# blyssprivacy/sdk

Measured on NVIDIA H100. Metric: PIR server queries/sec (Spiral process_query), higher is better.
Workload: dtype u64

## Files before the change

sdk_b200/csrc/api.cu:

```cuda
#include "../../include/b200pir.h"
#include "kernels.h"
#include "ntt_tables.hpp"
#include "update_body.hpp"
#include "dpir_wire.hpp"
#include "gadget.hpp"
#include <cstdio>
#include <cerrno>
#include <fcntl.h>
#include <unistd.h>
#include <algorithm>
#include <cmath>
#include <memory>
#include <cstring>
#include <condition_variable>
#include <chrono>
#include <deque>
#include <mutex>
#include <set>
#include <string>
#include <utility>
#include <vector>

using namespace b200pir;

// ... 41 lines not shown
  void ensure(size_t count) { if (count > n) alloc(count); }
  void release() { if (p) cudaFree(p); p = nullptr; n = 0; }
  ~DevBuf() { release(); }
  DevBuf(const DevBuf&) = delete;
  DevBuf& operator=(const DevBuf&) = delete;
};

enum Stage { ST_EXPAND = 0, ST_MUL, ST_FROMNTT, ST_FOLD, ST_PACK, ST_ENCODE, ST_QIMG , ST_COUNT };

}

struct b200pir_ctx {
  int device = 0;
  cudaStream_t stream = nullptr;
  bool own_stream = true;
  std::recursive_mutex mu;
  b200pir_params hp;
  int dim0, num_per, slices, trials, g, stop_round, num_packing;
  int bits_gsw, bits_conv, bits_left, bits_right;
  int live_gsw, live_conv, live_left, live_right;
  bool has_right;
  uint64_t q2, q1, setup_bytes, query_bytes, response_bytes;
  int q1_bits;
  DevParams dp;
  DevBuf<Twiddle> d_tw;
  DevBuf<Twiddle> d_tw4k;
  DevBuf<uint32_t> d_neg1;
  int mul_variant = 0, max_group = 16, profile = 0;
  int sparse_fold = 0;
  int db_format = -1;
  DevBuf<uint2> w_qf;
  DevBuf<uint8_t> w_qt;
  int sm_count = 0;
  size_t ws_queries = 0, ws_rows = 0;
  DevBuf<uint64_t> w_query;
  DevBuf<uint32_t> w_v;
  DevBuf<uint32_t> w_zflags;
  DevBuf<uint32_t> w_xr;
  DevBuf<uint4> w_qdev;
  DevBuf<uint32_t> w_vfold, w_vfold_neg;
  DevBuf<uint32_t> w_mult;
  DevBuf<uint32_t> w_cts;
  const uint32_t* folded = nullptr;
  size_t folded_stride = 0;
  DevBuf<uint64_t> w_packed;
  DevBuf<uint8_t> w_resp;
  static constexpr size_t kWriteStageBytes = (size_t)64 << 20;
  static constexpr size_t kWriteStageItems = 65536;
  DevBuf<uint8_t> w_wbytes;
  DevBuf<ItemWrite> w_witems;
  std::mutex export_mu;
  uint8_t* h_export[2] = {nullptr, nullptr};
  size_t h_export_bytes = 0;
  cudaEvent_t export_done[2] = {nullptr, nullptr};
  void ensure_export_staging(size_t bytes) {
    w_wbytes.ensure(std::max(kWriteStageBytes, bytes));
    if (!export_done[0])
      for (auto& e : export_done) B200_CUDA(cudaEventCreateWithFlags(&e, cudaEventDisableTiming | cudaEventBlockingSync));
    if (bytes <= h_export_bytes) return;
    release_export_pinned();
    const size_t n = std::max(kWriteStageBytes, bytes);
    for (auto& h : h_export) B200_CUDA(cudaHostAlloc(reinterpret_cast<void**>(&h), n, cudaHostAllocDefault));
    h_export_bytes = n;
  }
  void release_export_pinned() {
    for (auto& h : h_export) { if (h) cudaFreeHost(h); h = nullptr; }
// ... 240 lines not shown
}

void run_expand_query(b200pir_ctx* c, b200pir_pp* pp, const uint64_t* query_raw, uint32_t* v, uint4* q_dev,
                      uint32_t* v_fold, int nq, uint8_t* images = nullptr) {
  const auto& hp = c->hp;
  cudaStream_t s = c->stream;
  launch_to_ntt_strided(c->dp, v, c->v_words(), query_raw, (size_t)2 * POLY, 2, nq, s);
  run_coefficient_expansion(c, pp, v, c->v_words(), nq, false);
  const int factor = hp.nu_2 > 0 ? 2 : 1;
  if (images) {
    const Tc5Geom T = make_tc5_geom(c->dim0, 32);
    for (int q0 = 0; q0 < nq; q0 += 16)
      launch_reorient_to_tc5(T, v + (size_t)q0 * c->v_words(), c->v_words(), factor, std::min(16, nq - q0),
                             images + (size_t)(q0 / 16) * tc5_query_bytes(T), s);
  } else {
    launch_reorient(c->geom(c->num_per), q_dev, (size_t)c->dim0 * POLY, v, c->v_words(), nq, factor, s);
  }
  if (hp.nu_2 > 0)
    launch_regev_to_gsw(c->dp, v_fold, c->fold_words(), v, c->v_words(), nq, (int)hp.nu_2, 2, 1, c->pp_table(pp, (size_t)nq).conv,
                        (int)hp.t_gsw, (int)hp.t_conv, c->bits_conv, c->live_conv, s);
}

void run_fold(b200pir_ctx* c, uint64_t* cts, size_t batch, size_t batch_stride, size_t num, int k0,
              const uint32_t* vfold, const uint32_t* vfold_neg, int slices_per_query) {
  const size_t mat = (size_t)2 * 2 * c->hp.t_gsw * 2 * POLY;
  int k = k0;
  for (size_t half = num / 2; half >= 1; half /= 2, k--) {
    launch_fold_round(c->dp, cts, batch, batch_stride, (int)half, vfold + (size_t)k * mat, vfold_neg + (size_t)k * mat,
                      c->fold_words(), slices_per_query, (int)c->hp.t_gsw, c->bits_gsw, c->stream);
  }
}

const uint32_t* run_fold_res(b200pir_ctx* c, uint32_t* a, uint32_t* b, size_t batch, size_t batch_stride, size_t num,
                             int k0, const uint32_t* vfold, int slices_per_query) {
  const size_t mat = (size_t)2 * 2 * c->hp.t_gsw * 2 * POLY;
  int k = k0;
  uint32_t* src = a;
  uint32_t* dst = b;
  uint32_t* zero_flags = nullptr;
  if (c->sparse_fold) {
    c->w_zflags.ensure(batch * num);
    zero_flags = c->w_zflags.p;
  }
  for (size_t half = num / 2; half >= 1; half /= 2, k--) {
    launch_fold_res(c->dp, src, dst, batch, batch_stride, (int)half, vfold + (size_t)k * mat, c->fold_words(),
                    slices_per_query, (int)c->hp.t_gsw, c->bits_gsw, c->live_gsw, zero_flags, c->stream);
    std::swap(src, dst);
  }
  return src;
}

void run_prepare(b200pir_ctx* c, b200pir_pp* pp, size_t count, bool images = false) {
  b200pir_ctx::Scope sc(c, ST_EXPAND);
  if (images) c->w_qt.ensure((count + 15) / 16 * tc5_query_bytes(make_tc5_geom(c->dim0, 32)));
  if (c->hp.expand_queries)
    run_expand_query(c, pp, c->w_query.p, c->w_v.p, c->w_qdev.p, c->w_vfold.p, (int)count, images ? c->w_qt.p : nullptr);
}

void run_first_dim(b200pir_ctx* c, b200pir_db* db, size_t count, const uint4* qdev, uint32_t* out, int slice_begin,
                   int slice_count, const uint8_t* images = nullptr, size_t per_group = 16) {
  const DbLayout& L = db->layout;
  const size_t q_stride = (size_t)c->dim0 * POLY;
  const size_t out_stride = (size_t)c->slices * db->rows * 4 * POLY;
  if (L.format == 0) {
    b200pir_ctx::Scope sc(c, ST_MUL);
    size_t qi = 0;
    while (qi < count) {
      int nq = 1;
      if (count - qi >= 4 && c->max_group >= 4) nq = 4;
      else if (count - qi >= 2 && c->max_group >= 2) nq = 2;
      launch_multiply(c->dp, L.G, reinterpret_cast<const uint4*>(L.base), qdev + qi * q_stride, out + qi * out_stride,
                      slice_begin, slice_count, nq, q_stride, out_stride, c->mul_variant, c->stream);
      c->mul_launches++;
      qi += nq;
    }
  } else if (L.format == 2) {
    if (!images) c->w_qt.ensure(tc5_query_bytes(L.T));
    const size_t step = images ? per_group : 16;
    for (size_t qi = 0, g = 0; qi < count; qi += step, g++) {
      const int nq = (int)std::min<size_t>(step, count - qi);
      const uint8_t* qt = images ? images + g * tc5_query_bytes(L.T) : c->w_qt.p;
      if (!images) {
        b200pir_ctx::Scope sq(c, ST_QIMG);
        launch_query_to_tc5(L.T, qdev + qi * q_stride, q_stride, nq, c->w_qt.p, c->stream);
      }
      b200pir_ctx::Scope sc(c, ST_MUL);
      launch_multiply_tc5(c->dp, L.T, L.base, db->tile_mask.p, qt, out + qi * out_stride, out_stride, nq, slice_begin,
                          slice_count, c->sm_count, c->stream);
      c->mul_launches++;
    }
  } else {
    c->w_qf.ensure(imma_query_cells(L.F));
    const size_t per_pass = (c->max_group >= 16 && imma_supports_16(L.F)) ? 16 : (c->max_group >= 8 ? 8 : 4);
    for (size_t qi = 0; qi < count; qi += per_pass) {
      const int nq = (int)std::min<size_t>(per_pass, count - qi);
      {
        b200pir_ctx::Scope sq(c, ST_QIMG);
        launch_query_to_frag(L.F, qdev + qi * q_stride, q_stride, nq, c->w_qf.p, c->stream);
      }
      {
        b200pir_ctx::Scope sc(c, ST_MUL);
        launch_multiply_imma(c->dp, L.F, reinterpret_cast<const uint4*>(L.base), c->w_qf.p, out + qi * out_stride, out_stride,
                             nq, slice_begin, slice_count, c->stream);
        c->mul_launches++;
      }
    }
  }
}

void run_first_dim_and_fold(b200pir_ctx* c, b200pir_db* db, size_t count, const uint4* qdev = nullptr,
                            const uint32_t* vfold = nullptr, const uint8_t* images = nullptr, size_t per_group = 16) {
  if (!qdev) qdev = c->w_qdev.p;
  if (!vfold) vfold = c->w_vfold.p;
  const int rows = db->rows;
  const size_t out_stride = (size_t)c->slices * rows * 4 * POLY;
  const bool zmajor = db->zmajor_product();
  run_first_dim(c, db, count, qdev, zmajor ? c->w_cts.p : c->w_mult.p, 0, c->slices, images, per_group);
  {
    b200pir_ctx::Scope sc(c, ST_FROMNTT);
    if (zmajor) launch_intt_from_zmajor(c->dp, db->layout.F, c->w_cts.p, out_stride, c->w_mult.p, (int)count, c->slices, c->stream);
    else launch_ntt32(c->dp, c->w_mult.p, count * c->slices * rows * 2, true, c->stream);
  }
  {
    b200pir_ctx::Scope sc(c, ST_FOLD);
    c->folded = c->w_mult.p;
    c->folded_stride = (size_t)rows * 4 * POLY;
    if (rows > 1)
      c->folded = run_fold_res(c, c->w_mult.p, c->w_cts.p, count * c->slices, (size_t)rows * 4 * POLY, rows,
                               (int)c->hp.nu_2 - 1, vfold, c->slices);
  }
}

void run_pack_encode(b200pir_ctx* c, b200pir_pp* pp, const uint32_t* folded, size_t ct_stride, size_t count,
                     uint8_t* out_dev) {
  const auto& hp = c->hp;
  const size_t packed_words = (size_t)hp.instances * (hp.n + 1) * hp.n * POLY;
  {
    b200pir_ctx::Scope sc(c, ST_PACK);
    launch_pack(c->dp, c->w_packed.p, packed_words, folded, ct_stride, (size_t)c->slices * ct_stride, (int)count, c->pp_table(pp, count).pack,
                (int)hp.n, (int)hp.instances, (int)hp.t_conv, c->bits_conv, c->live_conv, (int)hp.version, c->stream);
  }
  {
    b200pir_ctx::Scope sc(c, ST_ENCODE);
    launch_encode(c->dp, out_dev, c->response_bytes, c->w_packed.p, packed_words, (int)count, (int)hp.n, (int)hp.instances,
                  c->q2, (int)hp.q2_bits, c->q1, c->q1_bits, c->stream);
  }
}

bool same_params(const b200pir_ctx* a, const b200pir_ctx* b) {
  return a == b || (a->device == b->device && std::memcmp(&a->hp, &b->hp, sizeof(b200pir_params)) == 0);
}
void check_db(b200pir_ctx* c, b200pir_db* db) {
  if (!db || !same_params(db->ctx, c)) throw Error(B200PIR_E_BADARG, "db handle was created for different parameters / device");
}
void check_pp(b200pir_ctx* c, b200pir_pp* pp) {
  if (!pp || !same_params(pp->ctx, c)) throw Error(B200PIR_E_BADARG, "pp handle was created for different parameters / device");
}

}

extern "C" {

// ... 89 lines not shown
  dp.q[0] = (uint32_t)q0; dp.q[1] = (uint32_t)q1m;
  dp.cr1[0] = (uint64_t)(((u128)1 << 64) / q0);
  dp.cr1[1] = (uint64_t)(((u128)1 << 64) / q1m);
  dp.modulus = q0 * q1m;
  dp.cr1_mod = (uint64_t)(((u128)1 << 64) / dp.modulus);
  dp.q1_inv_mod_q0 = (uint32_t)invmod(q1m % q0, q0);
  dp.fwd[0] = c->d_tw.p; dp.inv[0] = c->d_tw.p + POLY; dp.fwd[1] = c->d_tw.p + 2 * POLY; dp.inv[1] = c->d_tw.p + 3 * POLY;
  dp.inv_lz[0] = c->d_tw.p + 4 * POLY; dp.inv_lz[1] = c->d_tw.p + 5 * POLY;
  dp.mu58[0] = (uint32_t)(((uint64_t)1 << 58) / q0); dp.mu58[1] = (uint32_t)(((uint64_t)1 << 58) / q1m);
  {
    std::vector<uint32_t> h((size_t)NTT_LOG_N * 2 * POLY, 0);
    for (int i = 0; i < NTT_LOG_N; i++) {
      int idx = POLY - (1 << i);
      h[((size_t)i * 2 + 0) * POLY + idx] = (uint32_t)(q0 - 1);
      h[((size_t)i * 2 + 1) * POLY + idx] = (uint32_t)(q1m - 1);
    }
    c->d_neg1.alloc(h.size());
    B200_CUDA(cudaMemcpy(c->d_neg1.p, h.data(), h.size() * 4, cudaMemcpyHostToDevice));
    launch_ntt32(dp, c->d_neg1.p, NTT_LOG_N, false, c->stream);
    B200_CUDA(cudaStreamSynchronize(c->stream));
  }
  B200_CUDA(cudaGetLastError());
  *out = c.release();
  API_END
}

void b200pir_ctx_destroy(b200pir_ctx* c) {
  if (!c) return;
  cudaSetDevice(c->device);
  cudaDeviceSynchronize();
  for (auto e : c->event_pool) cudaEventDestroy(e);
  c->release_export_pinned();
  for (auto e : c->export_done) if (e) cudaEventDestroy(e);
  if (c->own_stream && c->stream) cudaStreamDestroy(c->stream);
  delete c;
}
int b200pir_ctx_set_stream(b200pir_ctx* c, void* cuda_stream) {
  API_BEGIN
  if (!c) throw Error(B200PIR_E_BADARG, "null ctx");
  Guard gd(c);
  B200_CUDA(cudaStreamSynchronize(c->stream));
  if (c->own_stream && c->stream) cudaStreamDestroy(c->stream);
  c->stream = (cudaStream_t)cuda_stream;
  c->own_stream = false;
  API_END
}
int b200pir_ctx_synchronize(b200pir_ctx* c) {
  API_BEGIN
  if (!c) throw Error(B200PIR_E_BADARG, "null ctx");
  Guard gd(c);
  B200_CUDA(cudaStreamSynchronize(c->stream));
  B200_CUDA(cudaGetLastError());
  API_END
}
int b200pir_ctx_reserve(b200pir_ctx* c, size_t queries, size_t rows_local) {
  API_BEGIN
  if (!c) throw Error(B200PIR_E_BADARG, "null ctx");
  if (queries == 0 || queries > 4096 || rows_local == 0 || rows_local > ((size_t)1 << c->hp.nu_2))
    throw Error(B200PIR_E_BADARG, "reserve: 1..4096 queries, 1..num_per rows");
  Guard gd(c);
  B200_CUDA(cudaStreamSynchronize(c->stream));
  c->ensure_workspace(queries, rows_local);
  B200_CUDA(cudaGetLastError());
  API_END
}
int b200pir_ctx_set_option(b200pir_ctx* c, const char* key, int64_t value) {
  API_BEGIN
  if (!c || !key) throw Error(B200PIR_E_BADARG, "null argument");
  Guard gd(c);
  std::string k(key);
  if (k == "mul_variant") c->mul_variant = (int)value;
  else if (k == "batch") { if (value != 1 && value != 2 && value != 4 && value != 8 && value != 16) throw Error(B200PIR_E_BADARG, "batch must be 1, 2, 4, 8 or 16"); c->max_group = (int)value; }
  else if (k == "fold_variant" || k == "intt_variant" || k == "imma_variant" || k == "expand_variant" ||
           k == "expand_pair_min_ctas") {}
  else if (k == "sparse_fold") c->sparse_fold = value != 0;
  else if (k == "coalesce") c->coalesce = value != 0;
  else if (k == "coalesce_window_us") { if (value < 0 || value > 100000) throw Error(B200PIR_E_BADARG, "coalesce_window_us must be 0..100000"); c->coalesce_window_us = (int)value; }
  else if (k == "db_format") { if (value < -1 || value > 2) throw Error(B200PIR_E_BADARG, "db_format must be -1 (automatic), 0, 1 or 2"); c->db_format = (int)value; }
  else if (k == "profile") {
    if (value < 0 || value > 2) throw Error(B200PIR_E_BADARG, "profile must be 0, 1 or 2");
    c->profile = (int)value;
    c->spans.clear(); c->event_next = 0; c->mul_launches = 0;
  }
  else throw Error(B200PIR_E_BADARG, "unknown option " + k);
  API_END
}
int b200pir_ctx_sizes(b200pir_ctx* c, uint64_t* setup_bytes, uint64_t* query_bytes, uint64_t* response_bytes) {
  API_BEGIN
  if (!c) throw Error(B200PIR_E_BADARG, "null ctx");
  if (setup_bytes) *setup_bytes = c->setup_bytes;
  if (query_bytes) *query_bytes = c->query_bytes;
  if (response_bytes) *response_bytes = c->response_bytes;
  API_END
}

int b200pir_db_create(b200pir_ctx* c, uint64_t shard_index, uint64_t shard_count, b200pir_db** out) {
  API_BEGIN
  if (!c || !out) throw Error(B200PIR_E_BADARG, "null argument");
  Guard gd(c);
  if (shard_count == 0) { shard_count = 1; shard_index = 0; }
  if (shard_index >= shard_count || (shard_count & (shard_count - 1)) || (uint64_t)c->num_per % shard_count)
    throw Error(B200PIR_E_BADARG, "shard_count must be a power of two dividing num_per");
  std::unique_ptr<b200pir_db> db(new b200pir_db());
  db->ctx = c;
  db->shard = Shard{(int)shard_index, (int)shard_count};
  db->rows = c->num_per / (int)shard_count;
  DbLayout& L = db->layout;
  L.G = c->geom(db->rows);
// ... 472 lines not shown
  if (count == 0) return 0;
  DevBuf<uint64_t> d(count * 2 * POLY);
  B200_CUDA(cudaMemcpyAsync(d.p, polys, d.n * 8, cudaMemcpyHostToDevice, c->stream));
  launch_ntt_u64(c->dp, d.p, count, inverse, c->stream);
  B200_CUDA(cudaMemcpyAsync(polys, d.p, d.n * 8, cudaMemcpyDeviceToHost, c->stream));
  B200_CUDA(cudaStreamSynchronize(c->stream));
  B200_CUDA(cudaGetLastError());
  API_END
}
int b200pir_ntt_forward(b200pir_ctx* c, uint64_t* polys, size_t count) { return ntt_host(c, polys, count, false); }
int b200pir_ntt_inverse(b200pir_ctx* c, uint64_t* polys, size_t count) { return ntt_host(c, polys, count, true); }

int b200pir_ntt32_dev(b200pir_ctx* c, uint32_t* polys_dev, size_t count, int inverse) {
  API_BEGIN
  if (!c || !polys_dev) throw Error(B200PIR_E_BADARG, "null argument");
  Guard gd(c);
  launch_ntt32(c->dp, polys_dev, count, inverse != 0, c->stream);
  B200_CUDA(cudaGetLastError());
  API_END
}

namespace {
const Twiddle* tables_4k(b200pir_ctx* c) {
  if (!c->d_tw4k.p) {
    const int N = 4096, LG = 12;
    std::vector<Twiddle> all;
    for (int n = 0; n < 2; n++) {
      std::vector<Twiddle> f, i;
      build_tables(c->dp.q[n], f, i, N, LG);
      all.insert(all.end(), f.begin(), f.end());
      all.insert(all.end(), i.begin(), i.end());
    }
    c->d_tw4k.alloc(all.size());
    B200_CUDA(cudaMemcpy(c->d_tw4k.p, all.data(), all.size() * sizeof(Twiddle), cudaMemcpyHostToDevice));
  }
  return c->d_tw4k.p;
}
}
int b200pir_ntt4096_dev(b200pir_ctx* c, uint32_t* polys_dev, size_t count, int inverse) {
  API_BEGIN
  if (!c || !polys_dev) throw Error(B200PIR_E_BADARG, "null argument");
  Guard gd(c);
  launch_ntt32_4k(c->dp.q[0], c->dp.q[1], tables_4k(c), polys_dev, count, inverse != 0, c->stream);
  B200_CUDA(cudaGetLastError());
  API_END
}
int b200pir_ntt4096(b200pir_ctx* c, uint64_t* polys, size_t count, int inverse) {
  API_BEGIN
  if (!c || (!polys && count)) throw Error(B200PIR_E_BADARG, "null argument");
  Guard gd(c);
  if (count == 0) return 0;
  const size_t words = count * 2 * 4096;
  DevBuf<uint64_t> wide(words);
  DevBuf<uint32_t> nar(words);
  B200_CUDA(cudaMemcpyAsync(wide.p, polys, words * 8, cudaMemcpyHostToDevice, c->stream));
  launch_narrow(nar.p, wide.p, words, c->stream);
  launch_ntt32_4k(c->dp.q[0], c->dp.q[1], tables_4k(c), nar.p, count, inverse != 0, c->stream);
  launch_widen(wide.p, nar.p, words, c->stream);
  B200_CUDA(cudaMemcpyAsync(polys, wide.p, words * 8, cudaMemcpyDeviceToHost, c->stream));
  B200_CUDA(cudaStreamSynchronize(c->stream));
  B200_CUDA(cudaGetLastError());
  API_END
}

int b200pir_to_ntt(b200pir_ctx* c, uint64_t* out_ntt, const uint64_t* raw, size_t count) {
  API_BEGIN
  if (!c || !out_ntt || !raw) throw Error(B200PIR_E_BADARG, "null argument");
// ... 1234 lines not shown
```

sdk_b200/csrc/kernels.h:

```cpp
#pragma once
#include "common.cuh"
#include "item_place.cuh"

namespace b200pir {

extern thread_local unsigned long long g_kernel_launches;

void opt_in_smem_impl(const void* kernel, int bytes);
template <typename K>
inline void opt_in_smem(K* kernel, int bytes) { opt_in_smem_impl(reinterpret_cast<const void*>(kernel), bytes); }

void launch_ntt_u64(const DevParams& P, uint64_t* polys, size_t count, bool inverse, cudaStream_t s);
void launch_ntt32(const DevParams& P, uint32_t* polys, size_t count, bool inverse, cudaStream_t s);
void launch_ntt32_4k(uint32_t q0, uint32_t q1, const Twiddle* tw, uint32_t* polys, size_t count, bool inverse, cudaStream_t s);
void launch_to_ntt(const DevParams& P, uint32_t* out, const uint64_t* raw, size_t count, cudaStream_t s);
void launch_to_ntt_strided(const DevParams& P, uint32_t* out, size_t out_stride, const uint64_t* raw, size_t raw_stride,
                           size_t count, int batches, cudaStream_t s);
void launch_chacha_first_rows(uint64_t* raw, const uint8_t seed[32], uint64_t word0, uint32_t n_mats, uint32_t row_words,
                              uint64_t mat_words, uint64_t modulus, cudaStream_t s);
void launch_direct_query_to_dev(uint4* q_dev, const uint32_t* sig_ntt, const uint64_t* wire_words, int dim0, cudaStream_t s);
void launch_from_ntt(const DevParams& P, uint64_t* out_raw, const uint32_t* in, size_t count, cudaStream_t s);
void launch_raw_to_res(const DevParams& P, uint32_t* out, const uint64_t* raw, size_t polys, cudaStream_t s);
void launch_res_to_raw(const DevParams& P, uint64_t* out, const uint32_t* res, size_t polys, cudaStream_t s);
void upload_poly_constants(const Twiddle* lo );
void upload_mul_constants(const Twiddle* lo );
void launch_widen(uint64_t* out, const uint32_t* in, size_t words, cudaStream_t s);
void launch_narrow(uint32_t* out, const uint64_t* in, size_t words, cudaStream_t s);

void launch_multiply(const DevParams& P, const MulGeom& G, const uint4* db_dev, const uint4* q_dev, uint32_t* out,
                     int slice_begin, int slice_count, int nq, size_t q_stride, size_t out_stride, int variant,
                     cudaStream_t s);
void launch_query_to_dev(const MulGeom& G, uint4* q_dev, const uint64_t* v_firstdim, cudaStream_t s);
struct Shard { int index, count; };
void launch_db_retile_chunk(const MulGeom& G, Shard sh, uint4* db_dev_slice, const uint64_t* ref_chunk, int z0, int zc,
                            cudaStream_t s);
void launch_db_synth(const DevParams& P, const MulGeom& G, Shard sh, uint4* db_dev, uint64_t seed, uint64_t pt_modulus,
                     int slice_begin, int slice_count, cudaStream_t s);

size_t imma_query_cells(const ImmaGeom& F);
bool imma_supports_16(const ImmaGeom& F);
inline int imma_query_tiles(int nq) { return nq > 8 ? 4 : (nq > 4 ? 2 : 1); }
void upload_imma_constants(const Twiddle* lo);
void launch_db_to_frag(const ImmaGeom& F, const uint4* db0_slice, uint4* dbf, int slice, cudaStream_t s);
void launch_query_to_frag(const ImmaGeom& F, const uint4* q_dev, size_t q_stride, int nq, uint2* qf, cudaStream_t s);
void launch_multiply_imma(const DevParams& P, const ImmaGeom& F, const uint4* dbf, const uint2* qf, uint32_t* out_zm,
                          size_t out_stride, int nq, int slice_begin, int slice_count, cudaStream_t s);
void launch_intt_from_zmajor(const DevParams& P, const ImmaGeom& F, const uint32_t* in_zm, size_t in_stride, uint32_t* out,
                             int nq, int slices, cudaStream_t s);
void launch_zmajor_to_ntt32(const ImmaGeom& F, const uint32_t* in_zm, uint32_t* out, int slice, cudaStream_t s);

size_t tc5_query_bytes(const Tc5Geom& T);
bool tc5_supported(const Tc5Geom& T);
void launch_db_to_tc5(const Tc5Geom& T, const uint4* db0_slice, uint8_t* dbt, int slice, cudaStream_t s);
void launch_query_to_tc5(const Tc5Geom& T, const uint4* q_dev, size_t q_stride, int nq, uint8_t* qt, cudaStream_t s);
void launch_reorient_to_tc5(const Tc5Geom& T, const uint32_t* v, size_t v_stride, int idx_factor, int nq, uint8_t* qt, cudaStream_t s);
void launch_multiply_tc5(const DevParams& P, const Tc5Geom& T, const uint8_t* dbt, const uint32_t* tile_mask, const uint8_t* qt,
                         uint32_t* out_zm, size_t out_stride, int nq, int slice_begin, int slice_count, int sm_count, cudaStream_t s);

void launch_db_upsert(const DbLayout& L, int slice, int il, int j, const uint64_t* poly, cudaStream_t s);
struct ItemWrite { uint32_t off, len, il, j; };
void launch_write_items(const DevParams& P, const DbLayout& L, const uint8_t* bytes, const ItemWrite* items, int count, int chunks,
                        int bpc, uint64_t pt_modulus, cudaStream_t s);
void launch_db_export(const DbLayout& L, int slice, int z0, int zc, uint64_t* out, cudaStream_t s);

void launch_fold_round(const DevParams& P, uint64_t* cts, size_t batch, size_t batch_stride , int half,
                       const uint32_t* c_pos, const uint32_t* c_neg, size_t c_batch_stride ,
                       int slices_per_query, int t_gsw, int bits, cudaStream_t s);
void launch_fold_res(const DevParams& P, const uint32_t* in, uint32_t* out, size_t batch, size_t batch_stride ,
                     int half, const uint32_t* c_pos, size_t c_batch_stride, int slices_per_query, int t_gsw, int bits, int live,
                     uint32_t* zero_flags , cudaStream_t s);
void launch_folding_neg(const DevParams& P, uint32_t* out, const uint32_t* v_folding, int count, int t_gsw, int bits,
                        cudaStream_t s);

struct PpTable { const uint32_t* const* pack; const uint32_t* const* left; const uint32_t* const* right; const uint32_t* const* conv; };
struct ExpandRound {
  int r, num_in, stop_round, max_bits_to_gen_right, t_auto;
  const uint32_t* const* tab_left;
  const uint32_t* const* tab_right;
  size_t off_left, off_right;
  int t_left, t_right, bits_left, bits_right;
  int live_left, live_right;
  int fill_skipped;
};
void launch_expand_round_res(const DevParams& P, uint32_t* v, size_t v_stride, uint32_t* xr, size_t xr_stride, int nq,
                             const ExpandRound& R, const uint32_t* neg1_r, cudaStream_t s);
void launch_reorient(const MulGeom& G, uint4* q_dev, size_t q_stride, const uint32_t* v, size_t v_stride, int nq,
                     int idx_factor, cudaStream_t s);
void launch_regev_to_gsw(const DevParams& P, uint32_t* v_gsw, size_t gsw_stride, const uint32_t* v, size_t v_stride,
                         int nq, int count, int idx_factor, int idx_offset, const uint32_t* const* tab_conv, int t_gsw,
                         int t_conv, int bits_conv, int live_conv, cudaStream_t s);
// ... 40 lines not shown
```

sdk_b200/csrc/tc5_kernels.cu:

```cuda
#include "kernels.h"
#include "item_place.cuh"
#include "tc5_ptx.cuh"

namespace b200pir {

namespace {

constexpr int TC5_SMEM_BUDGET = 227 * 1024 - 1024;
constexpr int TC5_THREADS = 2 * 128 + 32;

using namespace tc5;

__global__ void __launch_bounds__(256)
k_db_to_tc5(Tc5Geom T, const uint4* __restrict__ db0_slice, uint8_t* __restrict__ dbt, int slice) {
  const int z = blockIdx.x, mt = blockIdx.y, ks = blockIdx.z;
  const Tc5DbThread t = tc5_db_thread(threadIdx.x, mt, ks);
  const int half = T.dim0 >> 1;
  uint32_t res[2][4];
#pragma unroll
  for (int p = 0; p < 2; p++) {
    const int jp = t.jp0 + p;
    uint4 w = make_uint4(0, 0, 0, 0);
    if (t.ii < T.rows && jp < half) w = db0_slice[((size_t)t.ii * half + jp) * POLY + z];
    res[0][2 * p] = w.x; res[1][2 * p] = w.y; res[0][2 * p + 1] = w.z; res[1][2 * p + 1] = w.w;
// ... 48 lines not shown
  __syncthreads();
#pragma unroll
  for (int zz = 0; zz < 8; zz++)
#pragma unroll
    for (int n = 0; n < 2; n++) {
      uint4* dst = reinterpret_cast<uint4*>(qt + tc5_q_tile(T, n, z0 + zz, ks) * TC5_TILE);
      dst[threadIdx.x] = reinterpret_cast<const uint4*>(rimg + ((size_t)zz * 2 + n) * TC5_TILE)[threadIdx.x];
    }
}

constexpr int TC5_MAX_STAGES = 24;
struct Tc5Smem {
  uint64_t full[TC5_MAX_STAGES], empty[TC5_MAX_STAGES];
  uint64_t bfull[2], bempty[2];
};
__host__ __device__ inline int tc5_ring_stages(int ks, int ksps, int bbufs) {
  const int n = (TC5_SMEM_BUDGET - bbufs * ks * TC5_TILE) / (ksps * TC5_TILE);
  return n > TC5_MAX_STAGES ? TC5_MAX_STAGES : n;
}

template <int KSPS, int BBUFS>
__global__ void __launch_bounds__(TC5_THREADS, 1)
k_multiply_tc5(DevParams P, Tc5Geom T, const uint8_t* __restrict__ dbt, const uint8_t* __restrict__ qt,
               uint32_t* __restrict__ out_zm, size_t out_stride, int nq, int slice_begin, int slice_count,
               const uint32_t* __restrict__ tile_mask ) {
  constexpr int TC5_STAGE_BYTES = KSPS * TC5_TILE;
  const int TC5_STAGES = tc5_ring_stages(T.ks, KSPS, BBUFS);
  extern __shared__ __align__(1024) uint8_t tc5_smem[];
  uint8_t* smem_b = tc5_smem;
  uint8_t* smem_a = smem_b + (size_t)BBUFS * T.ks * TC5_TILE;
  Tc5Smem* S = reinterpret_cast<Tc5Smem*>(smem_a + (size_t)TC5_STAGES * TC5_STAGE_BYTES);
  const int warp = threadIdx.x >> 5, lane = threadIdx.x & 31;
  const int stages_per_tile = (T.ks + KSPS - 1) / KSPS;
  const int tiles_per_item = slice_count * T.mt;
  const int n_items = 2 * POLY;
  const uint32_t b_bytes = (uint32_t)T.ks * TC5_TILE;

  if (threadIdx.x == 0) {
    for (int s = 0; s < TC5_STAGES; s++) { mbar_init(&S->full[s], 1); mbar_init(&S->empty[s], 2); }
    for (int b = 0; b < 2; b++) { mbar_init(&S->bfull[b], 1); mbar_init(&S->bempty[b], 2); }
    asm volatile("fence.mbarrier_init.release.cluster;" ::: "memory");
  }
  __syncthreads();

  if (warp == 8) {
    int stage = 0; uint32_t sphase = 0;
    int it = 0;
    for (int item = blockIdx.x; item < n_items; item += gridDim.x, it++) {
      const int n = item & 1, z = item >> 1, bb = it % BBUFS;
      mbar_wait(&S->bempty[bb], ((it / BBUFS) & 1) ^ 1);
      if (elect_one()) {
        mbar_expect_tx(&S->bfull[bb], b_bytes);
        bulk_g2s(smem_b + (size_t)bb * b_bytes, qt + tc5_q_tile(T, n, z, 0) * TC5_TILE, b_bytes, &S->bfull[bb]);
      }
      __syncwarp();
      for (int sl = 0; sl < slice_count; sl++)
        for (int mt = 0; mt < T.mt; mt++) {
          const uint8_t* src = dbt + tc5_db_tile(T, slice_begin + sl, n, z, mt, 0) * TC5_TILE;
          const uint32_t mask = __ldg(tile_mask + (size_t)(slice_begin + sl) * T.mt + mt);
          for (int st = 0; st < stages_per_tile; st++) {
            const int ks_here = min(KSPS, T.ks - st * KSPS);
            const uint32_t full_m = ks_here == 32 ? 0xffffffffu : ((1u << ks_here) - 1u);
            const uint32_t km = (mask >> (st * KSPS)) & full_m;
            if (km == 0) continue;
            mbar_wait(&S->empty[stage], sphase ^ 1);
            if (elect_one()) {
              uint8_t* dst = smem_a + (size_t)stage * TC5_STAGE_BYTES;
              const uint8_t* from = src + (size_t)st * TC5_STAGE_BYTES;
              mbar_expect_tx(&S->full[stage], (uint32_t)__popc(km) * TC5_TILE);
              if (km == full_m) bulk_g2s(dst, from, (uint32_t)ks_here * TC5_TILE, &S->full[stage]);
              else
                for (int kk = 0; kk < ks_here; kk++)
                  if ((km >> kk) & 1u) bulk_g2s(dst + (size_t)kk * TC5_TILE, from + (size_t)kk * TC5_TILE, TC5_TILE, &S->full[stage]);
            }
            __syncwarp();
            if (++stage == TC5_STAGES) { stage = 0; sphase ^= 1; }
          }
        }
    }
  } else if (warp < 8) {
    const int wg = warp >> 2, w = warp & 3;
    const bool leader = (threadIdx.x & 127) == 0;
    int stage = 0; uint32_t sphase = 0;
    int it = 0;
    for (int item = blockIdx.x; item < n_items; item += gridDim.x, it++) {
      const int n = item & 1, z = item >> 1, bb = it % BBUFS;
      const uint32_t q = n ? P.q[1] : P.q[0];
      const Tc5Weights W = tc5_lane_weights(lane, q);
      mbar_wait(&S->bfull[bb], (it / BBUFS) & 1);
      const uint32_t b_addr = smem_u32(smem_b + (size_t)bb * b_bytes);
      for (int t = 0, slice = slice_begin, mt = 0; t < tiles_per_item; t++, mt++) {
        if (mt == T.mt) { mt = 0; slice++; }
        const uint32_t mask = __ldg(tile_mask + (size_t)slice * T.mt + mt);
        uint32_t acc[64];
#pragma unroll
        for (int c = 0; c < 64; c++) acc[c] = 0;
        int prev = -1;
        for (int st = 0; st < stages_per_tile; st++) {
          const int ks_here = min(KSPS, T.ks - st * KSPS);
          const uint32_t km = (mask >> (st * KSPS)) & (ks_here == 32 ? 0xffffffffu : ((1u << ks_here) - 1u));
          if (km == 0) continue;
          mbar_wait(&S->full[stage], sphase);
          const uint32_t a_addr = smem_u32(smem_a + (size_t)stage * TC5_STAGE_BYTES) + wg * (TC5_TILE / 2);
          wgmma_fence();
#pragma unroll
          for (int kk = 0; kk < KSPS; kk++)
            if ((km >> kk) & 1u)
              wgmma_m64n128k32_u8(acc, tc5_smem_desc(a_addr + kk * TC5_TILE), tc5_smem_desc(b_addr + (st * KSPS + kk) * TC5_TILE));
          wgmma_commit();
          wgmma_wait<1>();
          if (prev >= 0 && leader) mbar_arrive(&S->empty[prev]);
          prev = stage;
          if (++stage == TC5_STAGES) { stage = 0; sphase ^= 1; }
        }
        wgmma_wait<0>();
        wgmma_fence_operands(acc);
        if (prev >= 0 && leader) mbar_arrive(&S->empty[prev]);
        uint64_t p32[32], s16[16], k16[16], s8[8], k8[8], s4[4], k4[4];
#pragma unroll
        for (int i = 0; i < 16; i++)
#pragma unroll
          for (int h = 0; h < 2; h++) p32[2 * i + h] = tc5_lane_partial(acc[4 * i + 2 * h], acc[4 * i + 2 * h + 1], W.w, W.wp);
        tc5_rs_split<32>((lane >> tc5_rs_lane_bit(0)) & 1, p32, s16, k16);
#pragma unroll
// ... 11 lines not shown
            out_zm[(size_t)qi * out_stride + ((((size_t)slice * 2 + n) * POLY + z) * T.rows + ii) * 2 + tc5_frag_ctrow(lane)] =
                tc5_barrett57(k4[f], W.mu, q);
        }
      }
      if (leader) mbar_arrive(&S->bempty[bb]);
    }
  }
}

}

size_t tc5_query_bytes(const Tc5Geom& T) { return (size_t)2 * POLY * T.ks * TC5_TILE; }
static size_t tc5_smem_bytes(const Tc5Geom& T, int ksps, int bbufs) {
  return (size_t)bbufs * T.ks * TC5_TILE + (size_t)tc5_ring_stages(T.ks, ksps, bbufs) * ksps * TC5_TILE + sizeof(Tc5Smem) + 16;
}
bool tc5_supported(const Tc5Geom& T) { return T.dim0 % 2 == 0 && tc5_ring_stages(T.ks, 4, 1) >= 2; }

void launch_db_to_tc5(const Tc5Geom& T, const uint4* db0_slice, uint8_t* dbt, int slice, cudaStream_t s) {
  ++g_kernel_launches;
  k_db_to_tc5<<<dim3(POLY, T.mt, T.ks), 256, 0, s>>>(T, db0_slice, dbt, slice);
}
void launch_query_to_tc5(const Tc5Geom& T, const uint4* q_dev, size_t q_stride, int nq, uint8_t* qt, cudaStream_t s) {
  if (nq < 1 || nq > 16) throw Error(-2, "wgmma multiply: 1..16 queries per pass");
  ++g_kernel_launches;
  k_query_to_tc5<<<dim3(POLY / 2, T.ks), 256, 0, s>>>(T, q_dev, q_stride, nq, qt);
}
void launch_reorient_to_tc5(const Tc5Geom& T, const uint32_t* v, size_t v_stride, int idx_factor, int nq, uint8_t* qt, cudaStream_t s) {
  if (nq < 1 || nq > 16) throw Error(-2, "wgmma multiply: 1..16 queries per pass");
  ++g_kernel_launches;
  opt_in_smem(k_reorient_to_tc5, 16 * TC5_TILE);
  k_reorient_to_tc5<<<dim3(POLY / 8, T.ks), 256, 16 * TC5_TILE, s>>>(T, v, v_stride, idx_factor, nq, qt);
}
void launch_multiply_tc5(const DevParams& P, const Tc5Geom& T, const uint8_t* dbt, const uint32_t* tile_mask, const uint8_t* qt,
                         uint32_t* out_zm, size_t out_stride, int nq, int slice_begin, int slice_count, int sm_count, cudaStream_t s) {
  if (nq < 1 || nq > 16) throw Error(-2, "wgmma multiply: 1..16 queries per pass");
  if (!tc5_supported(T)) throw Error(-2, "wgmma multiply: dim0 too large for one CTA's shared memory");
  ++g_kernel_launches;
  const int grid = sm_count > 0 ? (sm_count < 2 * POLY ? sm_count : 2 * POLY) : 132;
  int ksps = 8, bbufs = 2;
  if (tc5_ring_stages(T.ks, ksps, bbufs) < 2) ksps = 4;
  if (tc5_ring_stages(T.ks, ksps, bbufs) < 2) bbufs = 1;
  const size_t smem = tc5_smem_bytes(T, ksps, bbufs);
#define TC5_LAUNCH(K, B)                                                                                                       \
  do {                                                                                                                         \
    opt_in_smem(k_multiply_tc5<K, B>, 227 * 1024);                                                                             \
    k_multiply_tc5<K, B><<<grid, TC5_THREADS, smem, s>>>(P, T, dbt, qt, out_zm, out_stride, nq, slice_begin, slice_count, tile_mask); \
  } while (0)
  if (ksps == 4) { if (bbufs == 2) TC5_LAUNCH(4, 2); else TC5_LAUNCH(4, 1); }
  else { if (bbufs == 2) TC5_LAUNCH(8, 2); else TC5_LAUNCH(8, 1); }
#undef TC5_LAUNCH
}

}
```

Measured before the change: 1580.

## Split tail work items across CTAs and overlap iNTT/fold halves on side stream

The tc5 multiply kernel now splits the leftover work items (those that do not fill a whole wave of the grid) into tile segments, so the last wave is spread across all CTAs rather than leaving most of them idle. The first-dim pipeline splits the query batch in half and runs the second half's iNTT and fold on a side stream synchronized by events, which aims to let the two halves run concurrently. New knobs for CTA count, slice groups and B-buffer count are also added. The side stream adds event overhead and partial-tile segments reload the query B tile for each segment.

```diff
diff --git a/sdk_b200/csrc/api.cu b/sdk_b200/csrc/api.cu
--- a/sdk_b200/csrc/api.cu
+++ b/sdk_b200/csrc/api.cu
@@ -97,6 +97,17 @@
   DevBuf<uint2> w_qf;
   DevBuf<uint8_t> w_qt;
   int sm_count = 0;
+  int first_dim_ctas = 0;
+  int first_dim_slice_groups = 0;
+  int first_dim_bbufs = 0;
+  cudaStream_t side_stream = nullptr;
+  cudaEvent_t side_begin = nullptr, side_end = nullptr;
+  void ensure_side_stream() {
+    if (side_stream) return;
+    B200_CUDA(cudaStreamCreateWithFlags(&side_stream, cudaStreamNonBlocking));
+    B200_CUDA(cudaEventCreateWithFlags(&side_begin, cudaEventDisableTiming));
+    B200_CUDA(cudaEventCreateWithFlags(&side_end, cudaEventDisableTiming));
+  }
   size_t ws_queries = 0, ws_rows = 0;
   DevBuf<uint64_t> w_query;
   DevBuf<uint32_t> w_v;
@@ -403,19 +414,21 @@
 }
 
 const uint32_t* run_fold_res(b200pir_ctx* c, uint32_t* a, uint32_t* b, size_t batch, size_t batch_stride, size_t num,
-                             int k0, const uint32_t* vfold, int slices_per_query) {
+                             int k0, const uint32_t* vfold, int slices_per_query, cudaStream_t st = nullptr,
+                             size_t flags_at = 0) {
+  if (!st) st = c->stream;
   const size_t mat = (size_t)2 * 2 * c->hp.t_gsw * 2 * POLY;
   int k = k0;
   uint32_t* src = a;
   uint32_t* dst = b;
   uint32_t* zero_flags = nullptr;
   if (c->sparse_fold) {
-    c->w_zflags.ensure(batch * num);
-    zero_flags = c->w_zflags.p;
+    c->w_zflags.ensure((flags_at + batch) * num);
+    zero_flags = c->w_zflags.p + flags_at * num;
   }
   for (size_t half = num / 2; half >= 1; half /= 2, k--) {
     launch_fold_res(c->dp, src, dst, batch, batch_stride, (int)half, vfold + (size_t)k * mat, c->fold_words(),
-                    slices_per_query, (int)c->hp.t_gsw, c->bits_gsw, c->live_gsw, zero_flags, c->stream);
+                    slices_per_query, (int)c->hp.t_gsw, c->bits_gsw, c->live_gsw, zero_flags, st);
     std::swap(src, dst);
   }
   return src;
@@ -448,6 +461,7 @@
   } else if (L.format == 2) {
     if (!images) c->w_qt.ensure(tc5_query_bytes(L.T));
     const size_t step = images ? per_group : 16;
+    const int groups = std::max(1, std::min(c->first_dim_slice_groups, slice_count));
     for (size_t qi = 0, g = 0; qi < count; qi += step, g++) {
       const int nq = (int)std::min<size_t>(step, count - qi);
       const uint8_t* qt = images ? images + g * tc5_query_bytes(L.T) : c->w_qt.p;
@@ -456,8 +470,11 @@
         launch_query_to_tc5(L.T, qdev + qi * q_stride, q_stride, nq, c->w_qt.p, c->stream);
       }
       b200pir_ctx::Scope sc(c, ST_MUL);
-      launch_multiply_tc5(c->dp, L.T, L.base, db->tile_mask.p, qt, out + qi * out_stride, out_stride, nq, slice_begin,
-                          slice_count, c->sm_count, c->stream);
+      for (int sg = 0; sg < groups; sg++) {
+        const int s0 = slice_begin + sg * slice_count / groups, s1 = slice_begin + (sg + 1) * slice_count / groups;
+        launch_multiply_tc5(c->dp, L.T, L.base, db->tile_mask.p, qt, out + qi * out_stride, out_stride, nq, s0, s1 - s0,
+                            c->first_dim_ctas > 0 ? c->first_dim_ctas : c->sm_count, c->first_dim_bbufs, c->stream);
+      }
       c->mul_launches++;
     }
   } else {
@@ -487,18 +504,39 @@
   const size_t out_stride = (size_t)c->slices * rows * 4 * POLY;
   const bool zmajor = db->zmajor_product();
   run_first_dim(c, db, count, qdev, zmajor ? c->w_cts.p : c->w_mult.p, 0, c->slices, images, per_group);
+  const size_t h = zmajor && count >= 2 ? count / 2 : count;
+  cudaStream_t side = nullptr;
+  if (h < count) {
+    c->ensure_side_stream();
+    side = c->side_stream;
+    if (c->sparse_fold && rows > 1) c->w_zflags.ensure(count * c->slices * rows);
+    B200_CUDA(cudaEventRecord(c->side_begin, c->stream));
+    B200_CUDA(cudaStreamWaitEvent(side, c->side_begin, 0));
+  }
   {
     b200pir_ctx::Scope sc(c, ST_FROMNTT);
-    if (zmajor) launch_intt_from_zmajor(c->dp, db->layout.F, c->w_cts.p, out_stride, c->w_mult.p, (int)count, c->slices, c->stream);
+    if (zmajor) launch_intt_from_zmajor(c->dp, db->layout.F, c->w_cts.p, out_stride, c->w_mult.p, (int)h, c->slices, c->stream);
     else launch_ntt32(c->dp, c->w_mult.p, count * c->slices * rows * 2, true, c->stream);
   }
+  if (side)
+    launch_intt_from_zmajor(c->dp, db->layout.F, c->w_cts.p + h * out_stride, out_stride, c->w_mult.p + h * out_stride,
+                            (int)(count - h), c->slices, side);
   {
     b200pir_ctx::Scope sc(c, ST_FOLD);
     c->folded = c->w_mult.p;
     c->folded_stride = (size_t)rows * 4 * POLY;
-    if (rows > 1)
-      c->folded = run_fold_res(c, c->w_mult.p, c->w_cts.p, count * c->slices, (size_t)rows * 4 * POLY, rows,
+    if (rows > 1) {
+      c->folded = run_fold_res(c, c->w_mult.p, c->w_cts.p, h * c->slices, (size_t)rows * 4 * POLY, rows,
                                (int)c->hp.nu_2 - 1, vfold, c->slices);
+      if (side)
+        run_fold_res(c, c->w_mult.p + h * out_stride, c->w_cts.p + h * out_stride, (count - h) * c->slices,
+                     (size_t)rows * 4 * POLY, rows, (int)c->hp.nu_2 - 1, vfold + h * c->fold_words(), c->slices, side,
+                     h * c->slices);
+    }
+    if (side) {
+      B200_CUDA(cudaEventRecord(c->side_end, side));
+      B200_CUDA(cudaStreamWaitEvent(c->stream, c->side_end, 0));
+    }
   }
 }
 
@@ -654,6 +692,11 @@
   for (auto e : c->event_pool) cudaEventDestroy(e);
   c->release_export_pinned();
   for (auto e : c->export_done) if (e) cudaEventDestroy(e);
+  if (c->side_stream) {
+    cudaEventDestroy(c->side_begin);
+    cudaEventDestroy(c->side_end);
+    cudaStreamDestroy(c->side_stream);
+  }
   if (c->own_stream && c->stream) cudaStreamDestroy(c->stream);
   delete c;
 }
@@ -696,6 +739,9 @@
   else if (k == "fold_variant" || k == "intt_variant" || k == "imma_variant" || k == "expand_variant" ||
            k == "expand_pair_min_ctas") {}
   else if (k == "sparse_fold") c->sparse_fold = value != 0;
+  else if (k == "first_dim_ctas") { if (value < 0 || value > c->sm_count) throw Error(B200PIR_E_BADARG, "first_dim_ctas must be 0 (default) .. the SM count"); c->first_dim_ctas = (int)value; }
+  else if (k == "first_dim_slice_groups") { if (value < 0 || value > c->slices) throw Error(B200PIR_E_BADARG, "first_dim_slice_groups must be 0 (default) .. slices"); c->first_dim_slice_groups = (int)value; }
+  else if (k == "first_dim_bbufs") { if (value < 0 || value > 2) throw Error(B200PIR_E_BADARG, "first_dim_bbufs must be 0 (automatic), 1 or 2"); c->first_dim_bbufs = (int)value; }
   else if (k == "coalesce") c->coalesce = value != 0;
   else if (k == "coalesce_window_us") { if (value < 0 || value > 100000) throw Error(B200PIR_E_BADARG, "coalesce_window_us must be 0..100000"); c->coalesce_window_us = (int)value; }
   else if (k == "db_format") { if (value < -1 || value > 2) throw Error(B200PIR_E_BADARG, "db_format must be -1 (automatic), 0, 1 or 2"); c->db_format = (int)value; }
@@ -1234,7 +1280,8 @@
       all.insert(all.end(), i.begin(), i.end());
     }
     c->d_tw4k.alloc(all.size());
-    B200_CUDA(cudaMemcpy(c->d_tw4k.p, all.data(), all.size() * sizeof(Twiddle), cudaMemcpyHostToDevice));
+    B200_CUDA(cudaMemcpyAsync(c->d_tw4k.p, all.data(), all.size() * sizeof(Twiddle), cudaMemcpyHostToDevice, c->stream));
+    B200_CUDA(cudaStreamSynchronize(c->stream));
   }
   return c->d_tw4k.p;
 }
diff --git a/sdk_b200/csrc/kernels.h b/sdk_b200/csrc/kernels.h
--- a/sdk_b200/csrc/kernels.h
+++ b/sdk_b200/csrc/kernels.h
@@ -55,7 +55,8 @@
 void launch_query_to_tc5(const Tc5Geom& T, const uint4* q_dev, size_t q_stride, int nq, uint8_t* qt, cudaStream_t s);
 void launch_reorient_to_tc5(const Tc5Geom& T, const uint32_t* v, size_t v_stride, int idx_factor, int nq, uint8_t* qt, cudaStream_t s);
 void launch_multiply_tc5(const DevParams& P, const Tc5Geom& T, const uint8_t* dbt, const uint32_t* tile_mask, const uint8_t* qt,
-                         uint32_t* out_zm, size_t out_stride, int nq, int slice_begin, int slice_count, int sm_count, cudaStream_t s);
+                         uint32_t* out_zm, size_t out_stride, int nq, int slice_begin, int slice_count, int ctas, int bbufs,
+                         cudaStream_t s);
 
 void launch_db_upsert(const DbLayout& L, int slice, int il, int j, const uint64_t* poly, cudaStream_t s);
 struct ItemWrite { uint32_t off, len, il, j; };
diff --git a/sdk_b200/csrc/tc5_kernels.cu b/sdk_b200/csrc/tc5_kernels.cu
--- a/sdk_b200/csrc/tc5_kernels.cu
+++ b/sdk_b200/csrc/tc5_kernels.cu
@@ -104,8 +104,12 @@
   Tc5Smem* S = reinterpret_cast<Tc5Smem*>(smem_a + (size_t)TC5_STAGES * TC5_STAGE_BYTES);
   const int warp = threadIdx.x >> 5, lane = threadIdx.x & 31;
   const int stages_per_tile = (T.ks + KSPS - 1) / KSPS;
+  const int n_items = 2 * POLY;
   const int tiles_per_item = slice_count * T.mt;
-  const int n_items = 2 * POLY;
+  const int full_items = n_items - n_items % gridDim.x;
+  const int tail_seg = max(1, min(tiles_per_item, ((n_items - full_items) * tiles_per_item + (int)gridDim.x - 1) / (int)gridDim.x));
+  const int segs_per_item = (tiles_per_item + tail_seg - 1) / tail_seg;
+  const int n_segs = full_items + (n_items - full_items) * segs_per_item;
   const uint32_t b_bytes = (uint32_t)T.ks * TC5_TILE;
 
   if (threadIdx.x == 0) {
@@ -117,8 +121,10 @@
 
   if (warp == 8) {
     int stage = 0; uint32_t sphase = 0;
-    int it = 0;
-    for (int item = blockIdx.x; item < n_items; item += gridDim.x, it++) {
+    for (int seg = blockIdx.x, it = 0; seg < n_segs; seg += gridDim.x, it++) {
+      const int item = seg < full_items ? seg : full_items + (seg - full_items) / segs_per_item;
+      const int t0 = seg < full_items ? 0 : (seg - full_items) % segs_per_item * tail_seg;
+      const int t1 = seg < full_items ? tiles_per_item : min(tiles_per_item, t0 + tail_seg);
       const int n = item & 1, z = item >> 1, bb = it % BBUFS;
       mbar_wait(&S->bempty[bb], ((it / BBUFS) & 1) ^ 1);
       if (elect_one()) {
@@ -126,42 +132,44 @@
         bulk_g2s(smem_b + (size_t)bb * b_bytes, qt + tc5_q_tile(T, n, z, 0) * TC5_TILE, b_bytes, &S->bfull[bb]);
       }
       __syncwarp();
-      for (int sl = 0; sl < slice_count; sl++)
-        for (int mt = 0; mt < T.mt; mt++) {
-          const uint8_t* src = dbt + tc5_db_tile(T, slice_begin + sl, n, z, mt, 0) * TC5_TILE;
-          const uint32_t mask = __ldg(tile_mask + (size_t)(slice_begin + sl) * T.mt + mt);
-          for (int st = 0; st < stages_per_tile; st++) {
-            const int ks_here = min(KSPS, T.ks - st * KSPS);
-            const uint32_t full_m = ks_here == 32 ? 0xffffffffu : ((1u << ks_here) - 1u);
-            const uint32_t km = (mask >> (st * KSPS)) & full_m;
-            if (km == 0) continue;
-            mbar_wait(&S->empty[stage], sphase ^ 1);
-            if (elect_one()) {
-              uint8_t* dst = smem_a + (size_t)stage * TC5_STAGE_BYTES;
-              const uint8_t* from = src + (size_t)st * TC5_STAGE_BYTES;
-              mbar_expect_tx(&S->full[stage], (uint32_t)__popc(km) * TC5_TILE);
-              if (km == full_m) bulk_g2s(dst, from, (uint32_t)ks_here * TC5_TILE, &S->full[stage]);
-              else
-                for (int kk = 0; kk < ks_here; kk++)
-                  if ((km >> kk) & 1u) bulk_g2s(dst + (size_t)kk * TC5_TILE, from + (size_t)kk * TC5_TILE, TC5_TILE, &S->full[stage]);
-            }
-            __syncwarp();
-            if (++stage == TC5_STAGES) { stage = 0; sphase ^= 1; }
+      for (int t = t0; t < t1; t++) {
+        const int sl = t / T.mt, mt = t - sl * T.mt;
+        const uint8_t* src = dbt + tc5_db_tile(T, slice_begin + sl, n, z, mt, 0) * TC5_TILE;
+        const uint32_t mask = __ldg(tile_mask + (size_t)(slice_begin + sl) * T.mt + mt);
+        for (int st = 0; st < stages_per_tile; st++) {
+          const int ks_here = min(KSPS, T.ks - st * KSPS);
+          const uint32_t full_m = ks_here == 32 ? 0xffffffffu : ((1u << ks_here) - 1u);
+          const uint32_t km = (mask >> (st * KSPS)) & full_m;
+          if (km == 0) continue;
+          mbar_wait(&S->empty[stage], sphase ^ 1);
+          if (elect_one()) {
+            uint8_t* dst = smem_a + (size_t)stage * TC5_STAGE_BYTES;
+            const uint8_t* from = src + (size_t)st * TC5_STAGE_BYTES;
+            mbar_expect_tx(&S->full[stage], (uint32_t)__popc(km) * TC5_TILE);
+            if (km == full_m) bulk_g2s(dst, from, (uint32_t)ks_here * TC5_TILE, &S->full[stage]);
+            else
+              for (int kk = 0; kk < ks_here; kk++)
+                if ((km >> kk) & 1u) bulk_g2s(dst + (size_t)kk * TC5_TILE, from + (size_t)kk * TC5_TILE, TC5_TILE, &S->full[stage]);
           }
+          __syncwarp();
+          if (++stage == TC5_STAGES) { stage = 0; sphase ^= 1; }
         }
+      }
     }
   } else if (warp < 8) {
     const int wg = warp >> 2, w = warp & 3;
     const bool leader = (threadIdx.x & 127) == 0;
     int stage = 0; uint32_t sphase = 0;
-    int it = 0;
-    for (int item = blockIdx.x; item < n_items; item += gridDim.x, it++) {
+    for (int seg = blockIdx.x, it = 0; seg < n_segs; seg += gridDim.x, it++) {
+      const int item = seg < full_items ? seg : full_items + (seg - full_items) / segs_per_item;
+      const int t0 = seg < full_items ? 0 : (seg - full_items) % segs_per_item * tail_seg;
+      const int t1 = seg < full_items ? tiles_per_item : min(tiles_per_item, t0 + tail_seg);
       const int n = item & 1, z = item >> 1, bb = it % BBUFS;
       const uint32_t q = n ? P.q[1] : P.q[0];
       const Tc5Weights W = tc5_lane_weights(lane, q);
       mbar_wait(&S->bfull[bb], (it / BBUFS) & 1);
       const uint32_t b_addr = smem_u32(smem_b + (size_t)bb * b_bytes);
-      for (int t = 0, slice = slice_begin, mt = 0; t < tiles_per_item; t++, mt++) {
+      for (int t = t0, slice = slice_begin + t0 / T.mt, mt = t0 % T.mt; t < t1; t++, mt++) {
         if (mt == T.mt) { mt = 0; slice++; }
         const uint32_t mask = __ldg(tile_mask + (size_t)slice * T.mt + mt);
         uint32_t acc[64];
@@ -239,12 +247,13 @@
   k_reorient_to_tc5<<<dim3(POLY / 8, T.ks), 256, 16 * TC5_TILE, s>>>(T, v, v_stride, idx_factor, nq, qt);
 }
 void launch_multiply_tc5(const DevParams& P, const Tc5Geom& T, const uint8_t* dbt, const uint32_t* tile_mask, const uint8_t* qt,
-                         uint32_t* out_zm, size_t out_stride, int nq, int slice_begin, int slice_count, int sm_count, cudaStream_t s) {
+                         uint32_t* out_zm, size_t out_stride, int nq, int slice_begin, int slice_count, int ctas, int bbufs_req,
+                         cudaStream_t s) {
   if (nq < 1 || nq > 16) throw Error(-2, "wgmma multiply: 1..16 queries per pass");
   if (!tc5_supported(T)) throw Error(-2, "wgmma multiply: dim0 too large for one CTA's shared memory");
   ++g_kernel_launches;
-  const int grid = sm_count > 0 ? (sm_count < 2 * POLY ? sm_count : 2 * POLY) : 132;
-  int ksps = 8, bbufs = 2;
+  const int grid = ctas > 0 ? (ctas < 2 * POLY ? ctas : 2 * POLY) : 132;
+  int ksps = 8, bbufs = bbufs_req == 1 ? 1 : 2;
   if (tc5_ring_stages(T.ks, ksps, bbufs) < 2) ksps = 4;
   if (tc5_ring_stages(T.ks, ksps, bbufs) < 2) bbufs = 1;
   const size_t smem = tc5_smem_bytes(T, ksps, bbufs);
```

Result: faster. 1599 (median of 6 runs) (+1.2%).
